# pythoncrazy/jimm

Hardware: AMD Instinct MI355X
Metric: images/sec (whole node) ViT-B/16@224 train (higher is better)
Workload: dtype bf16; 1 GPU; model=ViT-B/16@224, global_batch=1024, img_size=224, parallelism=dp1

## Files before the change

jimm_amd/csrc/attention.hip:

```cpp

#include <torch/extension.h>
#include <ATen/hip/HIPContext.h>

#include "mfma.h"

namespace {

constexpr int QBLK = 64;
constexpr int NSTRIP = 2;
constexpr int KVBLK = 64;


template <bool CAUSAL, int DP>
__global__ __launch_bounds__(256) void attn_fwd_kernel(
    const bf16* __restrict__ q, const bf16* __restrict__ k, const bf16* __restrict__ v,
    bf16* __restrict__ o, float* __restrict__ lse, int Lq, int Lk, float scale, int H, int Dr,
    hstride q_s, hstride k_s, hstride v_s, hstride o_s) {
  constexpr int LDS_PITCH = DP + 8;
  constexpr int NS = DP / 32;
  constexpr int NT = DP / 16;
  constexpr int IMGSF = KVBLK * LDS_PITCH + KVBLK * DP;
  extern __shared__ __attribute__((aligned(16))) char smem[];
  short* k_lds = reinterpret_cast<short*>(smem);
  short* vt_lds = k_lds + KVBLK * LDS_PITCH;
// ... 179 lines not shown
    float invl_r[4];
#pragma unroll
    for (int r = 0; r < 4; ++r) invl_r[r] = __shfl(invl, hi * 4 + r, WAVE);
#pragma unroll
    for (int r = 0; r < 4; ++r) {
      const int qrow = q0 + hi * 4 + r;
      if (qrow >= Lq) continue;
#pragma unroll
      for (int dt = 0; dt < NT; ++dt)
        if (DP == 64 || 16 * dt + lo < Dr)
          op[(int64_t)qrow * o_s.l + 16 * dt + lo] = f2bf(acc_o[st][dt][r] * invl_r[r]);
    }
    if (hi == 0 && q0 + lo < Lq)
      lse[bh * Lq + q0 + lo] = m_run[st] + __logf(l_run[st]);
  }
}


template <bool CAUSAL>
__global__ __launch_bounds__(320) void attn_fwd_small_kernel(
    const bf16* __restrict__ q, const bf16* __restrict__ k, const bf16* __restrict__ v,
    bf16* __restrict__ o, float* __restrict__ lse, int Lq, int Lk, float scale, int H,
    hstride q_s, hstride k_s, hstride v_s, hstride o_s) {
  constexpr int D = 64;
  constexpr int LP = 96;
  constexpr int PPITCH = 88;
  constexpr int PSTRIDE = 16 * PPITCH + 8;
  extern __shared__ __attribute__((aligned(16))) char smem[];
  const int wave = threadIdx.x / WAVE;
  const int lane = threadIdx.x % WAVE;
  const int lo = lane & 15, hi = lane >> 4;
  short* vb = reinterpret_cast<short*>(smem);
  short* pt = vb + LP * D + wave * PSTRIDE;

  const int64_t bh = blockIdx.x;
#pragma unroll
  for (int i = 0; i < (PSTRIDE / 8 + WAVE - 1) / WAVE; ++i) {
    const int idx = i * WAVE + lane;
    if (idx < PSTRIDE / 8) *reinterpret_cast<bf16x8*>(pt + idx * 8) = bf16x8{};
  }
  const bf16* qp = head_ptr(q, q_s, bh, H);
  const bf16* kp = head_ptr(k, k_s, bh, H);
  const bf16* vp = head_ptr(v, v_s, bh, H);
  bf16* op = head_ptr(o, o_s, bh, H);

  {
    const int t = (int)threadIdx.x;
    for (int idx = t; idx < LP * D / 8; idx += 320) {
      const int key = idx >> 3;
      const int d8 = (idx & 7) * 8;
      bf16x8 vv_{};
      if (key < Lk) vv_ = *reinterpret_cast<const bf16x8*>(vp + (int64_t)key * v_s.l + d8);
      *reinterpret_cast<bf16x8*>(vb + boff<D>(key, d8)) = vv_;
    }
  }
  const int nq = (Lq + 15) / 16;
  const int nkt = (Lk + 15) / 16;
  const int qs = wave;
  __syncthreads();
  if (qs < nq) {
    const int q0 = qs * 16;
    const int ktmax0 = CAUSAL ? min(nkt, qs + 1) : nkt;
    bf16x8 kfr[5][2];
#pragma unroll
    for (int kt = 0; kt < 5; ++kt) {
      const int key = 16 * kt + lo;
#pragma unroll
      for (int s = 0; s < 2; ++s)
        kfr[kt][s] = (kt < ktmax0 && key < Lk)
                         ? *reinterpret_cast<const bf16x8*>(kp + (int64_t)key * k_s.l + 32 * s + hi * 8)
                         : bf16x8{};
    }
    const int qrow = min(q0 + lo, Lq - 1);
    const bf16x8 qb0 = *reinterpret_cast<const bf16x8*>(qp + (int64_t)qrow * q_s.l + hi * 8);
    const bf16x8 qb1 = *reinterpret_cast<const bf16x8*>(qp + (int64_t)qrow * q_s.l + 32 + hi * 8);

    const int ktmax = ktmax0;
    f32x4 sc[5] = {};
    __builtin_amdgcn_s_setprio(1);
#pragma unroll
    for (int kt = 0; kt < 5; ++kt) {
      if (kt >= ktmax) continue;
      sc[kt] = MFMA16(kfr[kt][0], qb0, sc[kt]);
      sc[kt] = MFMA16(kfr[kt][1], qb1, sc[kt]);
    }
    __builtin_amdgcn_s_setprio(0);

    const int q_idx = q0 + lo;
    float sv[20];
#pragma unroll
    for (int kt = 0; kt < 5; ++kt) {
#pragma unroll
      for (int r = 0; r < 4; ++r) {
        const int key = 16 * kt + hi * 4 + r;
        float x = sc[kt][r] * scale;
        if (kt >= ktmax || key >= Lk || (CAUSAL && key > q_idx)) x = -INFINITY;
        sv[4 * kt + r] = x;
      }
    }
    float mt = sv[0];
#pragma unroll
    for (int i = 1; i < 20; ++i) mt = fmaxf(mt, sv[i]);
    mt = fmaxf(mt, __shfl_xor(mt, 16, WAVE));
    mt = fmaxf(mt, __shfl_xor(mt, 32, WAVE));
    float psum = 0.f;
#pragma unroll
    for (int i = 0; i < 20; ++i) {
      const float p = (sv[i] == -INFINITY) ? 0.f : __expf(sv[i] - mt);
      sv[i] = p;
      psum += p;
    }
    psum += __shfl_xor(psum, 16, WAVE);
    psum += __shfl_xor(psum, 32, WAVE);

#pragma unroll
    for (int kt = 0; kt < 5; ++kt) {
      bf16x4 pk;
#pragma unroll
      for (int r = 0; r < 4; ++r) pk[r] = f2bfs(sv[4 * kt + r]);
      *reinterpret_cast<bf16x4*>(pt + lo * PPITCH + 16 * kt + hi * 4) = pk;
    }

    f32x4 acc_o[4] = {};
    const int kv_hi = CAUSAL ? min(Lk, q0 + 16) : Lk;
#pragma unroll
    for (int s = 0; s < 3; ++s) {
      if (32 * s >= kv_hi) continue;
      bf16x8 vbf[4];
      const lds_cp bbase = (lds_cp)(const void*)(vb + s * 32 * D) + lane * 8;
      tr_frag_x4(bbase, vbf);
      const bf16x8 pa = row_frag(pt, lo, PPITCH, s, hi);
      __builtin_amdgcn_s_setprio(1);
#pragma unroll
      for (int dt = 0; dt < 4; ++dt) acc_o[dt] = MFMA16(pa, vbf[dt], acc_o[dt]);
      __builtin_amdgcn_s_setprio(0);
    }

    const float invl = psum > 0.f ? 1.f / psum : 0.f;
    float invl_r[4];
#pragma unroll
    for (int r = 0; r < 4; ++r) invl_r[r] = __shfl(invl, hi * 4 + r, WAVE);
#pragma unroll
    for (int r = 0; r < 4; ++r) {
      const int qr = q0 + hi * 4 + r;
      if (qr >= Lq) continue;
#pragma unroll
      for (int dt = 0; dt < 4; ++dt)
        op[(int64_t)qr * o_s.l + 16 * dt + lo] = f2bf(acc_o[dt][r] * invl_r[r]);
    }
    if (hi == 0 && q0 + lo < Lq) lse[bh * Lq + q0 + lo] = mt + __logf(psum);
  }
}

}

std::vector<torch::Tensor> attn_fwd(torch::Tensor q, torch::Tensor k, torch::Tensor v,
                                    bool causal, double scale) {
  check_attn_args("attn_fwd", {{"q", q}}, {{"k", k}, {"v", v}});
  const int Dr = q.size(3);
  const int DP = Dr <= 64 ? 64 : (Dr <= 96 ? 96 : 128);
  const int B = q.size(0), H = q.size(1), Lq = q.size(2), Lk = k.size(2);
  auto o = torch::empty({B, Lq, H, Dr}, q.options()).permute({0, 2, 1, 3});
  auto lse = torch::empty({B, H, Lq}, q.options().dtype(torch::kFloat32));
  const unsigned BH = (unsigned)((int64_t)B * H);
  auto stream = at::hip::getCurrentHIPStream();
  with_flags(
      [&](auto c) {
        constexpr bool C = decltype(c)::value;
        if (Dr == 64 && Lq == Lk && Lk <= 80) {
          const size_t shmem = (96 * 64 + 5 * (16 * 88 + 8)) * sizeof(short);
          launch_lds<attn_fwd_small_kernel<C>>(
              dim3(BH), dim3(320), shmem, shmem, stream, bf16_ptr(q), bf16_ptr(k), bf16_ptr(v),
              bf16_ptr(o), lse.data_ptr<float>(), Lq, Lk, (float)scale, H, hstrides(q),
              hstrides(k), hstrides(v), hstrides(o));
          return;
        }
        const int ntq = (Lq + QBLK - 1) / QBLK;
        const size_t shmem =
            (2 * (KVBLK * DP + KVBLK * (DP + 8)) + 4 * 16 * (DP + 8)) * sizeof(short);
        with_int<64, 96, 128>(DP, "padded head dim", [&](auto dp) {
          launch_lds<attn_fwd_kernel<C, decltype(dp)::value>>(
              dim3((ntq + NSTRIP - 1) / NSTRIP, BH), dim3(256), shmem, shmem, stream,
              bf16_ptr(q), bf16_ptr(k), bf16_ptr(v), bf16_ptr(o), lse.data_ptr<float>(), Lq, Lk,
              (float)scale, H, Dr, hstrides(q), hstrides(k), hstrides(v), hstrides(o));
        });
      },
      causal);
  return {o, lse};
}
```

jimm_amd/csrc/attention_bwd_fused.hip:

```cpp

#include <torch/extension.h>
#include <ATen/hip/HIPContext.h>

#include "mfma.h"

namespace {

constexpr int BLK = 64;

constexpr int tiles_per_wg(int DP) { return DP == 64 ? 2 : 1; }



__global__ void attn_d2_kernel(const bf16* __restrict__ dO, const bf16* __restrict__ O,
                               float* __restrict__ Dv, int H, int L, int Dr, int64_t nrows,
                               hstride do_s, hstride o_s) {
  const int wave = threadIdx.x / WAVE;
  const int lane = threadIdx.x % WAVE;
  const int wpb = blockDim.x / WAVE;
  const int sub = lane >> 3;
  const int c0 = (lane & 7) * 8;
  for (int64_t base = ((int64_t)blockIdx.x * wpb + wave) * 8; base < nrows;
       base += (int64_t)gridDim.x * wpb * 8) {
    const int64_t row = base + sub;
// ... 470 lines not shown
  const int64_t bh = blockIdx.x;
  const bf16* qp = head_ptr(q, q_s, bh, H);
  const bf16* kp = head_ptr(k, k_s, bh, H);
  const bf16* vp = head_ptr(v, v_s, bh, H);
  const bf16* dop = head_ptr(dO, do_s, bh, H);
  bf16* dqp = head_ptr(dq, dq_s, bh, H);
  bf16* dkp = head_ptr(dk, dk_s, bh, H);
  bf16* dvp = head_ptr(dv, dv_s, bh, H);

  for (int i = threadIdx.x; i < (3 * TILE + 8) / 8; i += 320)
    *reinterpret_cast<bf16x8*>(PT + i * 8) = bf16x8{};
  auto stage = [&](short* img, const bf16* src, int64_t sl, int rows) {
    for (int idx = (int)threadIdx.x; idx < IMG / 8; idx += 320) {
      const int row = idx >> 3, d8 = (idx & 7) * 8;
      bf16x8 vv{};
      if (row < rows) vv = *reinterpret_cast<const bf16x8*>(src + (int64_t)row * sl + d8);
      *reinterpret_cast<bf16x8*>(img + boff<D>(row, d8)) = vv;
    }
  };
  stage(imgA, kp, k_s.l, Lk);
  stage(imgQ, qp, q_s.l, Lq);
  stage(imgD, dop, do_s.l, Lq);
  const int nq = (Lq + 15) / 16;
  const int nkt = (Lk + 15) / 16;
  __syncthreads();

  if (wave < nq) {
    const int qs = wave;
    const int q0 = 16 * qs;
    const int ktmax = CAUSAL ? min(nkt, qs + 1) : nkt;
    bf16x8 kfr[5][2], vfr[5][2];
#pragma unroll
    for (int kt = 0; kt < 5; ++kt) {
      const int key = 16 * kt + lo;
      const bool ok = kt < ktmax && key < Lk;
#pragma unroll
      for (int sj = 0; sj < 2; ++sj) {
        kfr[kt][sj] = ok ? *reinterpret_cast<const bf16x8*>(
                               kp + (int64_t)key * k_s.l + 32 * sj + hi * 8)
                         : bf16x8{};
        vfr[kt][sj] = ok ? *reinterpret_cast<const bf16x8*>(
                               vp + (int64_t)key * v_s.l + 32 * sj + hi * 8)
                         : bf16x8{};
      }
    }
    const int qrow = min(q0 + lo, Lq - 1);
    const bf16x8 qb0 = *reinterpret_cast<const bf16x8*>(qp + (int64_t)qrow * q_s.l + hi * 8);
    const bf16x8 qb1 =
        *reinterpret_cast<const bf16x8*>(qp + (int64_t)qrow * q_s.l + 32 + hi * 8);
    const bf16x8 db0 =
        *reinterpret_cast<const bf16x8*>(dop + (int64_t)qrow * do_s.l + hi * 8);
    const bf16x8 db1 =
        *reinterpret_cast<const bf16x8*>(dop + (int64_t)qrow * do_s.l + 32 + hi * 8);
    f32x4 sc[5] = {}, dpc[5] = {};
    __builtin_amdgcn_s_setprio(1);
#pragma unroll
    for (int kt = 0; kt < 5; ++kt) {
      if (kt >= ktmax) continue;
      sc[kt] = MFMA16(kfr[kt][0], qb0, sc[kt]);
      sc[kt] = MFMA16(kfr[kt][1], qb1, sc[kt]);
      dpc[kt] = MFMA16(vfr[kt][0], db0, dpc[kt]);
      dpc[kt] = MFMA16(vfr[kt][1], db1, dpc[kt]);
    }
    __builtin_amdgcn_s_setprio(0);
    const int q_idx = q0 + lo;
    const float lse_q = lse[bh * Lq + qrow];
    float pv[20];
    float dsum = 0.f;
#pragma unroll
    for (int kt = 0; kt < 5; ++kt) {
#pragma unroll
      for (int r = 0; r < 4; ++r) {
        const int key = 16 * kt + 4 * hi + r;
        const bool ok =
            kt < ktmax && key < Lk && q_idx < Lq && (!CAUSAL || key <= q_idx);
        const float p = ok ? __expf(sc[kt][r] * scale - lse_q) : 0.f;
        pv[4 * kt + r] = p;
        dsum += p * dpc[kt][r];
      }
    }
    dsum += __shfl_xor(dsum, 16, WAVE);
    dsum += __shfl_xor(dsum, 32, WAVE);
#pragma unroll
    for (int kt = 0; kt < 5; ++kt) {
      bf16x4 ds4;
#pragma unroll
      for (int r = 0; r < 4; ++r) {
        const int key = 16 * kt + 4 * hi + r;
        const float p = pv[4 * kt + r];
        const float ds = p * (dpc[kt][r] - dsum) * scale;
        PT[key * TP + q_idx] = f2bfs(p);
        DST[key * TP + q_idx] = f2bfs(ds);
        ds4[r] = f2bfs(ds);
      }
      *reinterpret_cast<bf16x4*>(DSQ + q_idx * TP + 16 * kt + 4 * hi) = ds4;
    }
    f32x4 adq[4] = {};
    const int smax = (16 * ktmax + 31) / 32;
#pragma unroll
    for (int sb = 0; sb < 3; ++sb) {
      if (sb >= smax) continue;
      bf16x8 bfr[4];
      tr_frag_x4((lds_cp)(const void*)(imgA + sb * 32 * D) + lane * 8, bfr);
      const bf16x8 pa = row_frag(DSQ, q0 + lo, TP, sb, hi);
      __builtin_amdgcn_s_setprio(1);
#pragma unroll
      for (int dt = 0; dt < 4; ++dt) adq[dt] = MFMA16(pa, bfr[dt], adq[dt]);
      __builtin_amdgcn_s_setprio(0);
    }
#pragma unroll
    for (int r = 0; r < 4; ++r) {
      const int qr = q0 + 4 * hi + r;
      if (qr >= Lq) continue;
#pragma unroll
      for (int dt = 0; dt < 4; ++dt)
        dqp[(int64_t)qr * dq_s.l + 16 * dt + lo] = f2bf(adq[dt][r]);
    }
  }
  __syncthreads();

  if (wave < nkt) {
    const int k0 = 16 * wave;
    const int smin = CAUSAL ? k0 / 32 : 0;
    const int nsq = (Lq + 31) / 32;
    f32x4 adk[4] = {}, adv[4] = {};
    for (int sb = smin; sb < nsq; ++sb) {
      bf16x8 bq[4], bd[4];
      tr_frag_x4((lds_cp)(const void*)(imgQ + sb * 32 * D) + lane * 8, bq);
      tr_frag_x4((lds_cp)(const void*)(imgD + sb * 32 * D) + lane * 8, bd);
      const bf16x8 ak = row_frag(DST, k0 + lo, TP, sb, hi);
      const bf16x8 av = row_frag(PT, k0 + lo, TP, sb, hi);
      __builtin_amdgcn_s_setprio(1);
#pragma unroll
      for (int dt = 0; dt < 4; ++dt) {
        adk[dt] = MFMA16(ak, bq[dt], adk[dt]);
        adv[dt] = MFMA16(av, bd[dt], adv[dt]);
      }
      __builtin_amdgcn_s_setprio(0);
    }
#pragma unroll
    for (int r = 0; r < 4; ++r) {
      const int kr = k0 + 4 * hi + r;
      if (kr >= Lk) continue;
#pragma unroll
      for (int dt = 0; dt < 4; ++dt) {
        dkp[(int64_t)kr * dk_s.l + 16 * dt + lo] = f2bf(adk[dt][r]);
        dvp[(int64_t)kr * dv_s.l + 16 * dt + lo] = f2bf(adv[dt][r]);
      }
    }
  }
}


constexpr int RES_LMIN = 81;
constexpr int RES_LMAX = 256;

__device__ __forceinline__ int noff(int row, int d) {
  return (row >> 5) * 2048 + (d >> 4) * 512 + (row & 31) * 16 + (d & 15);
}

__global__ __launch_bounds__(512, 4) void attn_bwd_resident_kernel(
    const bf16* __restrict__ q, const bf16* __restrict__ k, const bf16* __restrict__ v,
    const bf16* __restrict__ o, const bf16* __restrict__ dO, const float* __restrict__ lse,
    bf16* __restrict__ dq, bf16* __restrict__ dk, bf16* __restrict__ dv, int L, float scale,
    int H, hstride q_s, hstride k_s, hstride v_s, hstride o_s, hstride do_s, hstride dq_s,
    hstride dk_s, hstride dv_s) {
  constexpr int D = 64;
  extern __shared__ __attribute__((aligned(16))) char smem[];
  const int LP = (L + 31) & ~31;
  const int IMG = LP * D;
  short* imgA = reinterpret_cast<short*>(smem);
  short* imgB = imgA + IMG;
  float* lse_s = reinterpret_cast<float*>(imgB + IMG);
  float* dl_s = lse_s + LP;

  const int tid = threadIdx.x;
  const int nthr = blockDim.x;
  const int nw = nthr / WAVE;
  const int wave = tid / WAVE;
  const int lane = tid % WAVE;
  const int lo = lane & 15, hi = lane >> 4;
  const int64_t bh = blockIdx.x;
  const bf16* qp = head_ptr(q, q_s, bh, H);
  const bf16* kp = head_ptr(k, k_s, bh, H);
  const bf16* vp = head_ptr(v, v_s, bh, H);
  const bf16* op = head_ptr(o, o_s, bh, H);
  const bf16* dop = head_ptr(dO, do_s, bh, H);
  const int nblk = LP / 32;

  bf16x8 qb[2], dob[2];
  float dl;
  auto load_rows = [&](int s0) {
    const int srow = min(s0 + lo, L - 1);
    dl = 0.f;
#pragma unroll
    for (int s = 0; s < 2; ++s) {
      qb[s] = *reinterpret_cast<const bf16x8*>(qp + (int64_t)srow * q_s.l + 32 * s + hi * 8);
      dob[s] = *reinterpret_cast<const bf16x8*>(dop + (int64_t)srow * do_s.l + 32 * s + hi * 8);
      const bf16x8 ov =
          *reinterpret_cast<const bf16x8*>(op + (int64_t)srow * o_s.l + 32 * s + hi * 8);
#pragma unroll
      for (int j = 0; j < 8; ++j) dl += bfs2f(dob[s][j]) * bfs2f(ov[j]);
    }
    dl += __shfl_xor(dl, 16, WAVE);
    dl += __shfl_xor(dl, 32, WAVE);
  };
  load_rows(16 * wave);

#pragma unroll
  for (int it = 0; it < 4; ++it) {
    const int idx = tid + it * nthr;
    const int row = idx >> 3, d8 = (idx & 7) * 8;
    const int rc = min(row, L - 1);
    bf16x8 kk = *reinterpret_cast<const bf16x8*>(kp + (int64_t)rc * k_s.l + d8);
    bf16x8 vv = *reinterpret_cast<const bf16x8*>(vp + (int64_t)rc * v_s.l + d8);
    if (row >= L) kk = vv = bf16x8{};
    const int off = noff(row, d8);
    *reinterpret_cast<bf16x8*>(imgA + off) = kk;
    *reinterpret_cast<bf16x8*>(imgB + off) = vv;
  }
  for (int i = tid; i < LP; i += nthr) {
    lse_s[i] = i < L ? lse[bh * L + i] : 0.f;
    dl_s[i] = 0.f;
  }
  __syncthreads();

#pragma unroll
  for (int i = 0; i < 2; ++i) {
    const int s0 = 16 * (wave + i * nw);
    if (s0 >= L) continue;
    if (i == 1) load_rows(s0);
    const bool sok = s0 + lo < L;
    const float lse_q = lse_s[min(s0 + lo, L - 1)];
    const float dli = dl;
    if (hi == 0) dl_s[s0 + lo] = dli;
    f32x4 adq[4] = {};
    for (int kb = 0; kb < nblk; ++kb) {
      f32x4 sc[2] = {}, dpc[2] = {};
#pragma unroll
      for (int t = 0; t < 2; ++t) {
        if (32 * kb + 16 * t >= L) continue;
        bf16x8 ka[2], va[2];
#pragma unroll
        for (int s = 0; s < 2; ++s) {
          const int off = noff(32 * kb + 16 * t + lo, 32 * s + hi * 8);
          ka[s] = *reinterpret_cast<const bf16x8*>(imgA + off);
          va[s] = *reinterpret_cast<const bf16x8*>(imgB + off);
        }
        __builtin_amdgcn_s_setprio(1);
#pragma unroll
        for (int s = 0; s < 2; ++s) {
          sc[t] = MFMA16(ka[s], qb[s], sc[t]);
          dpc[t] = MFMA16(va[s], dob[s], dpc[t]);
        }
        __builtin_amdgcn_s_setprio(0);
      }
      bf16x8 dsa;
#pragma unroll
      for (int t = 0; t < 2; ++t) {
#pragma unroll
        for (int r = 0; r < 4; ++r) {
          const int key = 32 * kb + 16 * t + 4 * hi + r;
          const bool ok = sok && key < L;
          const float p = ok ? __expf(sc[t][r] * scale - lse_q) : 0.f;
          const float ds = ok ? p * (dpc[t][r] - dli) * scale : 0.f;
          dsa[4 * t + r] = f2bfs(ds);
        }
      }
      bf16x8 bfr[4];
      tr_frag_x4((lds_cp)(const void*)(imgA + kb * 32 * D) + lane * 8, bfr);
      __builtin_amdgcn_s_setprio(1);
#pragma unroll
      for (int dt = 0; dt < 4; ++dt) adq[dt] = MFMA16(bfr[dt], dsa, adq[dt]);
      __builtin_amdgcn_s_setprio(0);
    }
    if (sok) {
      bf16* dqp = head_ptr(dq, dq_s, bh, H) + (int64_t)(s0 + lo) * dq_s.l + 4 * hi;
#pragma unroll
      for (int dt = 0; dt < 4; ++dt) {
        bf16x4 pk;
#pragma unroll
        for (int r = 0; r < 4; ++r) pk[r] = f2bfs(adq[dt][r]);
        *reinterpret_cast<bf16x4*>(dqp + 16 * dt) = pk;
      }
    }
  }

  bf16x8 qst[4], dst[4];
#pragma unroll
  for (int it = 0; it < 4; ++it) {
    const int idx = tid + it * nthr;
    const int row = idx >> 3, d8 = (idx & 7) * 8;
    const int rc = min(row, L - 1);
    qst[it] = *reinterpret_cast<const bf16x8*>(qp + (int64_t)rc * q_s.l + d8);
    dst[it] = *reinterpret_cast<const bf16x8*>(dop + (int64_t)rc * do_s.l + d8);
    if (row >= L) qst[it] = dst[it] = bf16x8{};
  }
  bf16x8 kbf[2][2], vbf[2][2];
#pragma unroll
  for (int i = 0; i < 2; ++i) {
    const int srow = min(16 * (wave + i * nw) + lo, LP - 1);
#pragma unroll
    for (int s = 0; s < 2; ++s) {
      const int off = noff(srow, 32 * s + hi * 8);
      kbf[i][s] = *reinterpret_cast<const bf16x8*>(imgA + off);
      vbf[i][s] = *reinterpret_cast<const bf16x8*>(imgB + off);
    }
  }
  __syncthreads();
#pragma unroll
  for (int it = 0; it < 4; ++it) {
    const int idx = tid + it * nthr;
    const int off = noff(idx >> 3, (idx & 7) * 8);
    *reinterpret_cast<bf16x8*>(imgA + off) = qst[it];
    *reinterpret_cast<bf16x8*>(imgB + off) = dst[it];
  }
  __syncthreads();

#pragma unroll
  for (int i = 0; i < 2; ++i) {
    const int s0 = 16 * (wave + i * nw);
    if (s0 >= L) continue;
    const bool sok = s0 + lo < L;
    f32x4 adk[4] = {}, adv[4] = {};
    for (int qblk = 0; qblk < nblk; ++qblk) {
      f32x4 sc[2] = {}, dpc[2] = {};
#pragma unroll
      for (int t = 0; t < 2; ++t) {
        if (32 * qblk + 16 * t >= L) continue;
        bf16x8 qa[2], da[2];
#pragma unroll
        for (int s = 0; s < 2; ++s) {
          const int off = noff(32 * qblk + 16 * t + lo, 32 * s + hi * 8);
          qa[s] = *reinterpret_cast<const bf16x8*>(imgA + off);
          da[s] = *reinterpret_cast<const bf16x8*>(imgB + off);
        }
        __builtin_amdgcn_s_setprio(1);
#pragma unroll
        for (int s = 0; s < 2; ++s) {
          sc[t] = MFMA16(qa[s], kbf[i][s], sc[t]);
          dpc[t] = MFMA16(da[s], vbf[i][s], dpc[t]);
        }
        __builtin_amdgcn_s_setprio(0);
      }
      bf16x8 pa, dsa;
#pragma unroll
      for (int t = 0; t < 2; ++t) {
        const int qi0 = 32 * qblk + 16 * t + 4 * hi;
        const f32x4 ls4 = *reinterpret_cast<const f32x4*>(lse_s + qi0);
        const f32x4 dl4 = *reinterpret_cast<const f32x4*>(dl_s + qi0);
#pragma unroll
        for (int r = 0; r < 4; ++r) {
          const bool ok = sok && qi0 + r < L;
          const float p = ok ? __expf(sc[t][r] * scale - ls4[r]) : 0.f;
          const float ds = ok ? p * (dpc[t][r] - dl4[r]) * scale : 0.f;
          pa[4 * t + r] = f2bfs(p);
          dsa[4 * t + r] = f2bfs(ds);
        }
      }
      bf16x8 bfr[4];
      tr_frag_x4((lds_cp)(const void*)(imgB + qblk * 32 * D) + lane * 8, bfr);
      __builtin_amdgcn_s_setprio(1);
#pragma unroll
      for (int dt = 0; dt < 4; ++dt) adv[dt] = MFMA16(bfr[dt], pa, adv[dt]);
      __builtin_amdgcn_s_setprio(0);
      tr_frag_x4((lds_cp)(const void*)(imgA + qblk * 32 * D) + lane * 8, bfr);
      __builtin_amdgcn_s_setprio(1);
#pragma unroll
      for (int dt = 0; dt < 4; ++dt) adk[dt] = MFMA16(bfr[dt], dsa, adk[dt]);
      __builtin_amdgcn_s_setprio(0);
    }
    if (sok) {
      bf16* dkp = head_ptr(dk, dk_s, bh, H) + (int64_t)(s0 + lo) * dk_s.l + 4 * hi;
      bf16* dvp = head_ptr(dv, dv_s, bh, H) + (int64_t)(s0 + lo) * dv_s.l + 4 * hi;
#pragma unroll
      for (int dt = 0; dt < 4; ++dt) {
        bf16x4 pk, pv;
#pragma unroll
        for (int r = 0; r < 4; ++r) {
          pk[r] = f2bfs(adk[dt][r]);
          pv[r] = f2bfs(adv[dt][r]);
        }
        *reinterpret_cast<bf16x4*>(dkp + 16 * dt) = pk;
        *reinterpret_cast<bf16x4*>(dvp + 16 * dt) = pv;
      }
    }
  }
}

}

void attn_bwd_fused(torch::Tensor q, torch::Tensor k, torch::Tensor v, torch::Tensor o,
                    torch::Tensor dO, torch::Tensor lse, torch::Tensor dq, torch::Tensor dk,
                    torch::Tensor dv, bool causal, double scale, std::string path) {
  check_attn_args("attn_bwd_fused", {{"q", q}, {"o", o}, {"dO", dO}, {"dq", dq}},
                  {{"k", k}, {"v", v}, {"dk", dk}, {"dv", dv}}, &lse);
  const int Dr = q.size(3);
  const int DP = Dr <= 64 ? 64 : (Dr <= 96 ? 96 : 128);
  const int B = q.size(0), H = q.size(1), Lq = q.size(2), Lk = k.size(2);
  const unsigned BH = (unsigned)((int64_t)B * H);
  auto stream = at::hip::getCurrentHIPStream();

  TORCH_CHECK(path == "auto" || path == "tiled" || path == "resident",
              "attn_bwd_fused: path must be auto, tiled or resident, got ", path);
  bool res_aligned = true;
  for (auto* t : {&q, &k, &v, &o, &dO, &dq, &dk, &dv})
    res_aligned = res_aligned && reinterpret_cast<uintptr_t>(t->data_ptr()) % 16 == 0 &&
                  t->stride(0) % 8 == 0 && t->stride(1) % 8 == 0 && t->stride(2) % 8 == 0;
  const bool resident_ok = Dr == 64 && Lq == Lk && !causal && Lk >= RES_LMIN &&
                           Lk <= RES_LMAX && res_aligned;
  TORCH_CHECK(path != "resident" || resident_ok,
              "attn_bwd_fused: path=resident needs D == 64, Lq == Lk, non-causal, ",
              RES_LMIN, " <= L <= ", RES_LMAX, " and 16-byte aligned rows; got D=", Dr,
              " Lq=", Lq, " Lk=", Lk, " causal=", causal, " aligned=", res_aligned);
  if (path != "tiled" && resident_ok) {
    const int LP = (Lk + 31) & ~31;
    const size_t rshmem = (size_t)2 * LP * 64 * sizeof(short) + (size_t)2 * LP * sizeof(float);
    constexpr size_t rshmem_max =
        (size_t)2 * RES_LMAX * 64 * sizeof(short) + (size_t)2 * RES_LMAX * sizeof(float);
    launch_lds<attn_bwd_resident_kernel>(
        dim3(BH), dim3(LP / 32 * WAVE), rshmem, rshmem_max, stream, bf16_ptr(q), bf16_ptr(k),
        bf16_ptr(v), bf16_ptr(o), bf16_ptr(dO), lse.data_ptr<float>(), bf16_ptr(dq),
        bf16_ptr(dk), bf16_ptr(dv), Lk, (float)scale, H, hstrides(q), hstrides(k), hstrides(v),
        hstrides(o), hstrides(dO), hstrides(dq), hstrides(dk), hstrides(dv));
    return;
  }

  if (path != "tiled" && Dr == 64 && Lq == Lk && Lk <= 80) {
    const size_t shmem = (3 * 96 * 64 + 3 * 80 * 88 + 8) * sizeof(short);
    with_flags(
        [&](auto c) {
          launch_lds<attn_bwd_small_kernel<decltype(c)::value>>(
              dim3(BH), dim3(320), shmem, shmem, stream, bf16_ptr(q), bf16_ptr(k), bf16_ptr(v),
              bf16_ptr(dO), lse.data_ptr<float>(), bf16_ptr(dq), bf16_ptr(dk), bf16_ptr(dv), Lq,
              Lk, (float)scale, H, hstrides(q), hstrides(k), hstrides(v), hstrides(dO),
              hstrides(dq), hstrides(dk), hstrides(dv));
        },
        causal);
    return;
  }

  auto Dv = torch::empty({(int64_t)B * H * Lq}, q.options().dtype(torch::kFloat32));
  {
    const int64_t nrows = (int64_t)B * H * Lq;
    const dim3 grid((unsigned)std::min<int64_t>((nrows + 3) / 4, 4096));
    hipLaunchKernelGGL(attn_d2_kernel, grid, dim3(256), 0, stream, bf16_ptr(dO), bf16_ptr(o),
                       Dv.data_ptr<float>(), H, Lq, Dr, nrows, hstrides(dO), hstrides(o));
  }

  const int pitch = DP + 8;
  const size_t shmem_dkv =
      (2 * (2 * BLK * DP + 2 * BLK * pitch) + 4 * 16 * pitch) * sizeof(short);
  const size_t shmem_dq = (2 * (BLK * DP + 2 * BLK * pitch) + 4 * 16 * pitch) * sizeof(short);
  const int ntk = (Lk + BLK - 1) / BLK;
  const int ntq = (Lq + BLK - 1) / BLK;
  const int tpw = tiles_per_wg(DP);
  with_flags(
      [&](auto c) {
        with_int<64, 96, 128>(DP, "padded head dim", [&](auto dp) {
          constexpr bool C = decltype(c)::value;
          constexpr int P = decltype(dp)::value;
          launch_lds<attn_bwd_dkv_kernel<C, P>>(
              dim3((ntk + tpw - 1) / tpw, BH), dim3(256), shmem_dkv, shmem_dkv, stream,
              bf16_ptr(q), bf16_ptr(k), bf16_ptr(v), bf16_ptr(dO), lse.data_ptr<float>(),
              Dv.data_ptr<float>(), bf16_ptr(dk), bf16_ptr(dv), Lq, Lk, (float)scale, H, Dr,
              hstrides(q), hstrides(k), hstrides(v), hstrides(dO), hstrides(dk), hstrides(dv));
          launch_lds<attn_bwd_dq_kernel<C, P>>(
              dim3((ntq + tpw - 1) / tpw, BH), dim3(256), shmem_dq, shmem_dq, stream,
              bf16_ptr(q), bf16_ptr(k), bf16_ptr(v), bf16_ptr(dO), lse.data_ptr<float>(),
              Dv.data_ptr<float>(), bf16_ptr(dq), Lq, Lk, (float)scale, H, Dr, hstrides(q),
              hstrides(k), hstrides(v), hstrides(dO), hstrides(dq));
        });
      },
      causal);
}
```

jimm_amd/csrc/bindings.cpp:

```cpp

#include <torch/extension.h>

std::vector<torch::Tensor> layernorm_fwd(torch::Tensor x, torch::Tensor w, torch::Tensor b, double eps);
std::vector<torch::Tensor> layernorm_bwd(torch::Tensor dy, torch::Tensor x, torch::Tensor w,
                                         torch::Tensor mean, torch::Tensor rstd,
                                         c10::optional<torch::Tensor> addend);
torch::Tensor bias_act_fwd(torch::Tensor z, c10::optional<torch::Tensor> bias, std::string act,
                           c10::optional<torch::Tensor> residual);
std::vector<torch::Tensor> bias_act_fwd_fp8(torch::Tensor z, c10::optional<torch::Tensor> bias,
                                            std::string act, torch::Tensor scale8,
                                            torch::Tensor amax);
std::vector<torch::Tensor> gemm_nt_8p_gradact_fp8(torch::Tensor dy, torch::Tensor wt,
                                                  torch::Tensor z, std::string act,
                                                  torch::Tensor scale8, torch::Tensor amax);
std::vector<torch::Tensor> layernorm_fwd_fp8(torch::Tensor x, torch::Tensor w, torch::Tensor b,
                                             double eps, torch::Tensor scale8,
                                             torch::Tensor amax);
torch::Tensor act_bwd(torch::Tensor dy, torch::Tensor z, std::string act);
torch::Tensor colsum(torch::Tensor dz);
torch::Tensor im2col_patch(torch::Tensor img, int64_t patch);
torch::Tensor cls_pos_fwd(torch::Tensor x, c10::optional<torch::Tensor> cls, torch::Tensor pos);
torch::Tensor embed_pos_fwd(torch::Tensor ids, torch::Tensor emb, torch::Tensor pos);
torch::Tensor col2im_patch(torch::Tensor cols, std::vector<int64_t> img_shape, int64_t patch);
void adam_step(std::vector<torch::Tensor> ps, std::vector<torch::Tensor> gs,
               std::vector<torch::Tensor> ms, std::vector<torch::Tensor> vs,
               std::vector<c10::optional<torch::Tensor>> masters, double lr, double b1,
               double b2, double eps, double wd, int64_t step);
std::vector<torch::Tensor> adam_prepare(std::vector<torch::Tensor> ps,
                                        std::vector<torch::Tensor> gs,
                                        std::vector<torch::Tensor> ms,
                                        std::vector<torch::Tensor> vs,
                                        std::vector<c10::optional<torch::Tensor>> masters);
void adam_apply(torch::Tensor desc, int64_t nchunks, torch::Tensor lr_dev,
                torch::Tensor step_dev, double b1, double b2, double eps, double wd);
std::vector<torch::Tensor> attn_fwd(torch::Tensor q, torch::Tensor k, torch::Tensor v,
                                    bool causal, double scale);
void attn_bwd_p(torch::Tensor s, torch::Tensor lse, bool causal, double scale);
torch::Tensor attn_d(torch::Tensor dO, torch::Tensor O);
void attn_ds(torch::Tensor dp, torch::Tensor p, torch::Tensor D, double scale);
void attn_bwd_fused(torch::Tensor q, torch::Tensor k, torch::Tensor v, torch::Tensor o,
                    torch::Tensor dO, torch::Tensor lse, torch::Tensor dq, torch::Tensor dk,
                    torch::Tensor dv, bool causal, double scale, std::string path);
torch::Tensor mfma_probe(torch::Tensor A, torch::Tensor B);
torch::Tensor mfma_probe32(torch::Tensor A, torch::Tensor B);
bool gemm_supported(int64_t M, int64_t N, int64_t K, std::string dtype);
std::vector<torch::Tensor> l2norm_fwd(torch::Tensor x);
torch::Tensor l2norm_bwd(torch::Tensor dy, torch::Tensor x, torch::Tensor rinv);
std::vector<torch::Tensor> xent_rows_fwd(torch::Tensor logits, torch::Tensor labels);
torch::Tensor xent_rows_bwd(torch::Tensor logits, torch::Tensor labels, torch::Tensor lse,
                            double gscale);
std::vector<torch::Tensor> sigmoid_loss_ew(torch::Tensor logits, int64_t diag0);
bool gemm8p_supported(int64_t M, int64_t N, int64_t K);
bool gemm_tn8p_supported(int64_t M, int64_t N, int64_t K);
int64_t gemm_tn8p_choose_splitm(int64_t M, int64_t tiles, int64_t cus);
torch::Tensor gemm_tn_8p(torch::Tensor dz, torch::Tensor x, int64_t splitm, bool out_bf16);
std::vector<torch::Tensor> gemm_tn_8p_db(torch::Tensor dz, torch::Tensor x, int64_t splitm,
                                         bool out_bf16);
torch::Tensor gemm_nt_8p_gradact(torch::Tensor dy, torch::Tensor wt, torch::Tensor z, std::string act);
torch::Tensor tr16_probe(torch::Tensor src, int64_t mode);
std::vector<torch::Tensor> linear_fwd(torch::Tensor x, torch::Tensor w,
                                      c10::optional<torch::Tensor> bias, std::string act,
                                      c10::optional<torch::Tensor> residual, bool save_z);
std::vector<torch::Tensor> linear_fwd_actgrad(torch::Tensor x, torch::Tensor w,
                                              c10::optional<torch::Tensor> bias,
                                              std::string act,
                                              c10::optional<torch::Tensor> residual);
torch::Tensor gemm_nt_8p_gradmul(torch::Tensor dy, torch::Tensor wt, torch::Tensor g);

PYBIND11_MODULE(TORCH_EXTENSION_NAME, m) {
  m.def("layernorm_fwd", &layernorm_fwd, "LayerNorm forward (K3)");
  m.def("layernorm_bwd", &layernorm_bwd, "LayerNorm backward (K3/K15), optional fused addend",
        py::arg("dy"), py::arg("x"), py::arg("w"), py::arg("mean"), py::arg("rstd"),
        py::arg("addend") = py::none());
  m.def("bias_act_fwd", &bias_act_fwd, "fused bias+activation(+residual) forward");
  m.def("bias_act_fwd_fp8", &bias_act_fwd_fp8, "bias+act forward with fused e4m3 emit");
  m.def("gemm_nt_8p_gradact_fp8", &gemm_nt_8p_gradact_fp8,
        "gradact dX GEMM with fused e4m3 emit of dz");
  m.def("layernorm_fwd_fp8", &layernorm_fwd_fp8, "LayerNorm forward with fused e4m3 emit");
  m.def("act_bwd", &act_bwd, "activation backward: dy * act'(z)");
  m.def("colsum", &colsum, "column sum -> fp32 (bias gradient, K15)");
  m.def("im2col_patch", &im2col_patch, "patch-embed unfold (K1)");
  m.def("cls_pos_fwd", &cls_pos_fwd, "fused CLS concat + pos-emb add (K2)");
  m.def("embed_pos_fwd", &embed_pos_fwd, "fused token-embed gather + pos-emb add (K10)");
  m.def("col2im_patch", &col2im_patch, "patch-embed fold backward (K1/K15)");
  m.def("adam_step", &adam_step, "fused multi-tensor Adam (K14)");
  m.def("adam_prepare", &adam_prepare, "build device chunk descriptors once (K14)");
  m.def("adam_apply", &adam_apply, "graph-capturable fused Adam update (K14)");
  m.def("attn_fwd", &attn_fwd, "flash attention forward, head_dim 64 (K5)");
  m.def("attn_bwd_p", &attn_bwd_p, "attention bwd: S -> P in place (K15)");
  m.def("attn_d", &attn_d, "attention bwd: rowsum(dO*O) (K15)");
  m.def("attn_ds", &attn_ds, "attention bwd: dP -> dS in place (K15)");
  m.def("attn_bwd_fused", &attn_bwd_fused,
        "fused flash attention backward (K15); path: auto | tiled | resident",
        py::arg("q"), py::arg("k"), py::arg("v"), py::arg("o"), py::arg("dO"), py::arg("lse"),
        py::arg("dq"), py::arg("dk"), py::arg("dv"), py::arg("causal"), py::arg("scale"),
        py::arg("path") = "auto");
  m.def("mfma_probe", &mfma_probe, "MFMA 16x16x32 layout probe");
  m.def("mfma_probe32", &mfma_probe32, "MFMA 32x32x16 layout probe");
  m.def("gemm_supported", &gemm_supported, "MFMA GEMM shape support check");
  m.def("gemm8p_supported", &gemm8p_supported, "8-phase 256-tile GEMM shape check");
  m.def("gemm_tn8p_supported", &gemm_tn8p_supported, "TN dW GEMM shape check");
  m.def("gemm_tn8p_choose_splitm", &gemm_tn8p_choose_splitm,
        "TN dW split-M heuristic (host only)", py::arg("M"), py::arg("tiles"), py::arg("cus"));
  m.def("gemm_tn_8p", &gemm_tn_8p, "TN weight-grad GEMM, split-M, tr_b16 (K15)",
        py::arg("dz"), py::arg("x"), py::arg("splitm") = 0, py::arg("out_bf16") = false);
  m.def("gemm_tn_8p_db", &gemm_tn_8p_db, "split-M TN dW with fused bias-grad colsum",
        py::arg("dz"), py::arg("x"), py::arg("splitm") = 0, py::arg("out_bf16") = false);
  m.def("gemm_nt_8p_gradact", &gemm_nt_8p_gradact, "dX GEMM with fused act-backward epilogue");
  m.def("tr16_probe", &tr16_probe, "ds_read_b64_tr_b16 lane-mapping probe");
  m.def("l2norm_fwd", &l2norm_fwd, "row L2-normalize forward (K12)");
  m.def("l2norm_bwd", &l2norm_bwd, "row L2-normalize backward (K12)");
  m.def("xent_rows_fwd", &xent_rows_fwd, "fused softmax-CE forward (K13)");
  m.def("xent_rows_bwd", &xent_rows_bwd, "fused softmax-CE backward (K13)");
  m.def("sigmoid_loss_ew", &sigmoid_loss_ew, "SigLIP sigmoid loss + dLogits (K13)");
  m.def("linear_fwd", &linear_fwd, "MFMA GEMM + fused epilogue (K4/K6/K7/K8)");
  m.def("linear_fwd_actgrad", &linear_fwd_actgrad,
        "linear_fwd that returns (y, fp16 act'(pre)) instead of the pre-activation",
        py::arg("x"), py::arg("w"), py::arg("bias"), py::arg("act"),
        py::arg("residual") = py::none());
  m.def("gemm_nt_8p_gradmul", &gemm_nt_8p_gradmul,
        "dX GEMM times a saved fp16 activation derivative");
}
```

jimm_amd/csrc/mfma.h:

```cpp
#pragma once

#include <string>
#include <type_traits>

#include "common.h"

#define MFMA16(A, B, C) __builtin_amdgcn_mfma_f32_16x16x32_bf16(A, B, C, 0, 0, 0)


__device__ __forceinline__ void raw_barrier() {
  asm volatile("s_barrier" ::: "memory");
}

__device__ __forceinline__ void glds16(const bf16* g, char* lds_dst) {
  typedef const __attribute__((address_space(1))) unsigned int* gp_t;
  typedef __attribute__((address_space(3))) unsigned int* lp_t;
  __builtin_amdgcn_global_load_lds((gp_t)(const void*)g, (lp_t)(void*)lds_dst, 16, 0, 0);
}

__device__ __forceinline__ int xcd_remap(int wg, int nwg) {
  const int q = nwg / 8, r = nwg % 8;
  const int xcd = wg % 8, idx = wg / 8;
  return (xcd < r ? xcd * (q + 1) : r * (q + 1) + (xcd - r) * q) + idx;
}

template <int DP>
__device__ __forceinline__ bf16x8 ld8g(const bf16* p, int off, int Dr) {
  if (DP == 64 || off + 8 <= Dr) return *reinterpret_cast<const bf16x8*>(p + off);
  return bf16x8{};
}

template <int ND>
__device__ __forceinline__ int boff(int q, int d) {
  const int qp = (q >> 2) & 7;
  const int qpos = (qp & 1) * 4 + (qp >> 1);
  return (q >> 5) * (32 * ND) + (d >> 4) * 512 + qpos * 64 + (q & 3) * 16 + (d & 15);
}

typedef const __attribute__((address_space(3))) char* lds_cp;

__device__ __forceinline__ void tr_frag_x4(lds_cp base, bf16x8 (&out)[4]) {
  bf16x4 a0l, a0h, a1l, a1h, a2l, a2h, a3l, a3h;
  asm volatile(
      "ds_read_b64_tr_b16 %0, %8 offset:0\n\t"
      "ds_read_b64_tr_b16 %1, %8 offset:512\n\t"
      "ds_read_b64_tr_b16 %2, %8 offset:1024\n\t"
      "ds_read_b64_tr_b16 %3, %8 offset:1536\n\t"
      "ds_read_b64_tr_b16 %4, %8 offset:2048\n\t"
      "ds_read_b64_tr_b16 %5, %8 offset:2560\n\t"
      "ds_read_b64_tr_b16 %6, %8 offset:3072\n\t"
      "ds_read_b64_tr_b16 %7, %8 offset:3584\n\t"
      "s_waitcnt lgkmcnt(0)"
      : "=&v"(a0l), "=&v"(a0h), "=&v"(a1l), "=&v"(a1h), "=&v"(a2l), "=&v"(a2h),
        "=&v"(a3l), "=&v"(a3h)
      : "v"(base)
      : "memory");
  __builtin_amdgcn_sched_barrier(0);
  out[0] = __builtin_shufflevector(a0l, a0h, 0, 1, 2, 3, 4, 5, 6, 7);
  out[1] = __builtin_shufflevector(a1l, a1h, 0, 1, 2, 3, 4, 5, 6, 7);
  out[2] = __builtin_shufflevector(a2l, a2h, 0, 1, 2, 3, 4, 5, 6, 7);
  out[3] = __builtin_shufflevector(a3l, a3h, 0, 1, 2, 3, 4, 5, 6, 7);
}

__device__ __forceinline__ void tr_frag_x2(lds_cp base, bf16x8 (&out)[2]) {
  bf16x4 a0l, a0h, a1l, a1h;
  asm volatile(
      "ds_read_b64_tr_b16 %0, %4 offset:0\n\t"
      "ds_read_b64_tr_b16 %1, %4 offset:512\n\t"
      "ds_read_b64_tr_b16 %2, %4 offset:1024\n\t"
      "ds_read_b64_tr_b16 %3, %4 offset:1536\n\t"
      "s_waitcnt lgkmcnt(0)"
      : "=&v"(a0l), "=&v"(a0h), "=&v"(a1l), "=&v"(a1h)
      : "v"(base)
      : "memory");
  __builtin_amdgcn_sched_barrier(0);
  out[0] = __builtin_shufflevector(a0l, a0h, 0, 1, 2, 3, 4, 5, 6, 7);
  out[1] = __builtin_shufflevector(a1l, a1h, 0, 1, 2, 3, 4, 5, 6, 7);
}

template <int NT>
__device__ __forceinline__ void tr_frags(lds_cp base, bf16x8 (&out)[NT]) {
  static_assert(NT == 4 || NT == 6 || NT == 8, "head dims 64, 96, 128");
  tr_frag_x4(base, *reinterpret_cast<bf16x8(*)[4]>(&out[0]));
  if constexpr (NT == 6) tr_frag_x2(base + 4096, *reinterpret_cast<bf16x8(*)[2]>(&out[4]));
  if constexpr (NT == 8) tr_frag_x4(base + 4096, *reinterpret_cast<bf16x8(*)[4]>(&out[4]));
}

__device__ __forceinline__ bf16x8 row_frag(const short* img, int row, int pitch, int step,
                                           int hi) {
  return *reinterpret_cast<const bf16x8*>(img + row * pitch + 32 * step + hi * 8);
}


struct hstride {
  int64_t b, h, l;
};

template <typename T>
__device__ __forceinline__ T* head_ptr(T* base, const hstride& s, int64_t bh, int H) {
  return base + (bh / H) * s.b + (bh % H) * s.h;
}


#define SAVE_NONE 0
#define SAVE_PRE 1
#define SAVE_GRAD 2

#define GRADM_NONE 0
#define GRADM_ACT 1
#define GRADM_MUL 2

__device__ __forceinline__ float load_bias(const void* bias, int n, int bias_bf16) {
  return bias_bf16 ? bf2f(static_cast<const bf16*>(bias)[n])
                   : static_cast<const float*>(bias)[n];
}

template <int ACT, bool HAS_BIAS, bool HAS_RES, int SAVE, int GRADM = GRADM_NONE,
          bool FP8O = false>
__device__ __forceinline__ void gemm_epilogue(float vpre, int m, int n, int N, float bias_n,
                                              const bf16* res, bf16* Y, bf16* Z,
                                              unsigned char* Y8 = nullptr, float rs8 = 1.f,
                                              float* tmax = nullptr) {
  static_assert(SAVE != SAVE_GRAD || ACT != ACT_NONE, "SAVE_GRAD needs an activation");
  if (HAS_BIAS) vpre += bias_n;
  if (SAVE == SAVE_PRE) Z[(int64_t)m * N + n] = f2bf(vpre);
  float vy;
  if (GRADM == GRADM_ACT) {
    vy = vpre * act_grad(bf2f(res[(int64_t)m * N + n]), ACT);
  } else if (GRADM == GRADM_MUL) {
    vy = vpre * __half2float(reinterpret_cast<const __half*>(res)[(int64_t)m * N + n]);
  } else {
    if (SAVE == SAVE_GRAD) {
      float g;
      vy = act_fwd_grad(vpre, ACT, &g);
      reinterpret_cast<__half*>(Z)[(int64_t)m * N + n] = __float2half(g);
    } else {
      vy = act_fwd(vpre, ACT);
    }
    if (HAS_RES) vy += bf2f(res[(int64_t)m * N + n]);
  }
  Y[(int64_t)m * N + n] = f2bf(vy);
  if (FP8O) {
    *tmax = fmaxf(*tmax, fabsf(vy));
    Y8[(int64_t)m * N + n] = cvt_e4m3(vy * rs8);
  }
}


int act_code(const std::string& act);

template <int... Vs, typename F>
void with_int(int v, const char* what, F&& f) {
  const bool found = ((v == Vs ? (f(std::integral_constant<int, Vs>{}), true) : false) || ...);
  TORCH_CHECK(found, "bad ", what, " ", v);
}

template <typename F>
void with_act(int act, F&& f) {
  with_int<ACT_NONE, ACT_GELU, ACT_GELU_TANH, ACT_QUICKGELU>(act, "activation code", f);
}

template <typename F>
void with_save(int save, F&& f) {
  with_int<SAVE_NONE, SAVE_PRE, SAVE_GRAD>(save, "save mode", f);
}

template <typename F>
void with_flags(F&& f) {
  f();
}
template <typename F, typename... Rest>
void with_flags(F&& f, bool b, Rest... rest) {
  if (b) with_flags([&](auto... cs) { f(std::true_type{}, cs...); }, rest...);
  else with_flags([&](auto... cs) { f(std::false_type{}, cs...); }, rest...);
}

template <auto Kernel, typename... Args>
void launch_lds(dim3 grid, dim3 block, size_t shmem, size_t shmem_limit, hipStream_t stream,
                Args... args) {
  static const bool raised = [&] {
    HIP_CHECK(hipFuncSetAttribute(reinterpret_cast<const void*>(Kernel),
                                  hipFuncAttributeMaxDynamicSharedMemorySize,
                                  (int)shmem_limit));
    return true;
  }();
  (void)raised;
  hipLaunchKernelGGL(Kernel, grid, block, shmem, stream, args...);
}


inline hstride hstrides(const torch::Tensor& t) {
  return {t.stride(0), t.stride(1), t.stride(2)};
}

inline bf16* bf16_ptr(const torch::Tensor& t) {
  return reinterpret_cast<bf16*>(t.data_ptr());
}

struct named_tensor {
  const char* name;
  const torch::Tensor& t;
};

inline void check_attn_args(const char* op, std::initializer_list<named_tensor> q_like,
                            std::initializer_list<named_tensor> k_like,
                            const torch::Tensor* lse = nullptr) {
  const torch::Tensor& q = q_like.begin()->t;
  const torch::Tensor& k = k_like.begin()->t;
  for (const auto* list : {&q_like, &k_like}) {
    const torch::Tensor& first = list->begin()->t;
    for (const named_tensor& n : *list) {
      TORCH_CHECK(n.t.is_cuda(), op, ": ", n.name, " must be a CUDA tensor");
      TORCH_CHECK(n.t.scalar_type() == torch::kBFloat16, op, ": ", n.name,
                  " must be bf16, got ", n.t.scalar_type());
      TORCH_CHECK(n.t.dim() == 4, op, ": ", n.name, " must be (B,H,L,D), got ", n.t.dim(),
                  " dims");
      TORCH_CHECK(n.t.stride(3) == 1, op, ": innermost dim of ", n.name,
                  " must be contiguous");
      TORCH_CHECK(n.t.sizes() == first.sizes(), op, ": ", n.name, " has shape ", n.t.sizes(),
                  ", expected ", list->begin()->name, "'s ", first.sizes());
    }
  }
  const int64_t D = q.size(3);
  TORCH_CHECK(D == 64 || D == 72 || D == 80 || D == 96 || D == 128, op,
              ": head_dim must be one of {64,72,80,96,128}, got ", D);
  TORCH_CHECK(k.size(0) == q.size(0) && k.size(1) == q.size(1) && k.size(3) == D, op,
              ": k has shape ", k.sizes(), ", expected q's B, H and D ", q.sizes());
  if (lse) {
    TORCH_CHECK(lse->is_cuda() && lse->is_contiguous() &&
                    lse->scalar_type() == torch::kFloat32 &&
                    lse->numel() == q.size(0) * q.size(1) * q.size(2),
                op, ": lse must be contiguous fp32 (B,H,Lq)");
  }
}
```

Measured before the change: 6610 images/sec.

## Add LDS-resident single-pass attention forward kernel for short sequences

Adds a forward attention kernel that loads a head's full K and V into LDS once and computes exact softmax in a single pass per 16-row query strip, with no online rescaling. It is used by default when head dim is 64, the sequence is non-causal and 81 to 256 long (ViT-B/16 has 197 tokens). The aim is to drop the tiled flash loop's repeated KV loads, running-max rescaling and multi-block bookkeeping. In exchange it keeps more score registers live, and occupancy is bounded by the LDS used for whole-head K and V. Shared helpers move into the common header.

Result: faster. 6757 images/sec, median of 6 (+2.2%).

```diff
diff --git a/jimm_amd/csrc/attention.hip b/jimm_amd/csrc/attention.hip
--- a/jimm_amd/csrc/attention.hip
+++ b/jimm_amd/csrc/attention.hip
@@ -355,18 +355,168 @@
   }
 }
 
+
+template <int NBLK>
+__global__ __launch_bounds__(512, 4) void attn_fwd_resident_kernel(
+    const bf16* __restrict__ q, const bf16* __restrict__ k, const bf16* __restrict__ v,
+    bf16* __restrict__ o, float* __restrict__ lse, int L, float scale, int H, hstride q_s,
+    hstride k_s, hstride v_s, hstride o_s) {
+  constexpr int D = 64;
+  constexpr int LP = 32 * NBLK;
+  constexpr int IMG = LP * D;
+  constexpr int NTHR = 64 * NBLK;
+  extern __shared__ __attribute__((aligned(16))) char smem[];
+  short* imgK = reinterpret_cast<short*>(smem);
+  short* imgV = imgK + IMG;
+
+  const int tid = threadIdx.x;
+  const int wave = tid / WAVE;
+  const int lane = tid % WAVE;
+  const int lo = lane & 15, hi = lane >> 4;
+  const int64_t bh = blockIdx.x;
+  const bf16* qp = head_ptr(q, q_s, bh, H);
+  const bf16* kp = head_ptr(k, k_s, bh, H);
+  const bf16* vp = head_ptr(v, v_s, bh, H);
+
+  bf16x8 qb[2][2];
+#pragma unroll
+  for (int i = 0; i < 2; ++i) {
+    const int srow = min(16 * (wave + i * NBLK) + lo, L - 1);
+#pragma unroll
+    for (int s = 0; s < 2; ++s)
+      qb[i][s] = *reinterpret_cast<const bf16x8*>(qp + (int64_t)srow * q_s.l + 32 * s + hi * 8);
+  }
+
+#pragma unroll
+  for (int it = 0; it < 4; ++it) {
+    const int idx = tid + it * NTHR;
+    const int row = idx >> 3, d8 = (idx & 7) * 8;
+    const int rc = min(row, L - 1);
+    bf16x8 kk = *reinterpret_cast<const bf16x8*>(kp + (int64_t)rc * k_s.l + d8);
+    bf16x8 vv = *reinterpret_cast<const bf16x8*>(vp + (int64_t)rc * v_s.l + d8);
+    if (row >= L) kk = vv = bf16x8{};
+    const int off = noff(row, d8);
+    *reinterpret_cast<bf16x8*>(imgK + off) = kk;
+    *reinterpret_cast<bf16x8*>(imgV + off) = vv;
+  }
+  __syncthreads();
+
+  const float c = scale * 1.44269504088896340736f;
+#pragma unroll
+  for (int i = 0; i < 2; ++i) {
+    const int s0 = 16 * (wave + i * NBLK);
+    if (s0 >= L) continue;
+    const bool sok = s0 + lo < L;
+
+    f32x4 sc[NBLK][2];
+#pragma unroll
+    for (int kb = 0; kb < NBLK; ++kb) {
+#pragma unroll
+      for (int t = 0; t < 2; ++t) {
+        sc[kb][t] = f32x4{};
+        if (kb == NBLK - 1 && 32 * kb + 16 * t >= L) continue;
+        bf16x8 ka[2];
+#pragma unroll
+        for (int s = 0; s < 2; ++s)
+          ka[s] = *reinterpret_cast<const bf16x8*>(
+              imgK + noff(32 * kb + 16 * t + lo, 32 * s + hi * 8));
+        __builtin_amdgcn_s_setprio(1);
+#pragma unroll
+        for (int s = 0; s < 2; ++s) sc[kb][t] = MFMA16(ka[s], qb[i][s], sc[kb][t]);
+        __builtin_amdgcn_s_setprio(0);
+      }
+    }
+
+    float m = -INFINITY;
+#pragma unroll
+    for (int kb = 0; kb < NBLK; ++kb) {
+#pragma unroll
+      for (int t = 0; t < 2; ++t) {
+#pragma unroll
+        for (int r = 0; r < 4; ++r) {
+          float x = sc[kb][t][r] * c;
+          if (kb == NBLK - 1 && 32 * kb + 16 * t + 4 * hi + r >= L) x = -INFINITY;
+          sc[kb][t][r] = x;
+          m = fmaxf(m, x);
+        }
+      }
+    }
+    m = fmaxf(m, __shfl_xor(m, 16, WAVE));
+    m = fmaxf(m, __shfl_xor(m, 32, WAVE));
+    const float msub = sok ? m : INFINITY;
+
+    float lsum = 0.f;
+    f32x4 acc[4] = {};
+#pragma unroll
+    for (int kb = 0; kb < NBLK; ++kb) {
+      bf16x8 pf;
+#pragma unroll
+      for (int t = 0; t < 2; ++t) {
+#pragma unroll
+        for (int r = 0; r < 4; ++r) {
+          const float p = __builtin_amdgcn_exp2f(sc[kb][t][r] - msub);
+          lsum += p;
+          pf[4 * t + r] = f2bfs(p);
+        }
+      }
+      bf16x8 vfr[4];
+      tr_frag_x4((lds_cp)(const void*)(imgV + kb * 32 * D) + lane * 8, vfr);
+      __builtin_amdgcn_s_setprio(1);
+#pragma unroll
+      for (int dt = 0; dt < 4; ++dt) acc[dt] = MFMA16(vfr[dt], pf, acc[dt]);
+      __builtin_amdgcn_s_setprio(0);
+    }
+    lsum += __shfl_xor(lsum, 16, WAVE);
+    lsum += __shfl_xor(lsum, 32, WAVE);
+
+    if (sok) {
+      const float invl = 1.f / lsum;
+      bf16* op = head_ptr(o, o_s, bh, H) + (int64_t)(s0 + lo) * o_s.l + 4 * hi;
+#pragma unroll
+      for (int dt = 0; dt < 4; ++dt) {
+        bf16x4 pk;
+#pragma unroll
+        for (int r = 0; r < 4; ++r) pk[r] = f2bfs(acc[dt][r] * invl);
+        *reinterpret_cast<bf16x4*>(op + 16 * dt) = pk;
+      }
+      if (hi == 0) lse[bh * L + s0 + lo] = m * 0.69314718055994530942f + __logf(lsum);
+    }
+  }
 }
 
+}
+
 std::vector<torch::Tensor> attn_fwd(torch::Tensor q, torch::Tensor k, torch::Tensor v,
-                                    bool causal, double scale) {
+                                    bool causal, double scale, std::string path) {
   check_attn_args("attn_fwd", {{"q", q}}, {{"k", k}, {"v", v}});
   const int Dr = q.size(3);
   const int DP = Dr <= 64 ? 64 : (Dr <= 96 ? 96 : 128);
   const int B = q.size(0), H = q.size(1), Lq = q.size(2), Lk = k.size(2);
+  TORCH_CHECK(path == "auto" || path == "tiled" || path == "resident",
+              "attn_fwd: path must be auto, tiled or resident, got ", path);
+  const bool aligned = res_aligned({&q, &k, &v});
+  const bool resident_ok = Dr == 64 && Lq == Lk && !causal && Lk >= RES_LMIN &&
+                           Lk <= RES_LMAX && aligned;
+  TORCH_CHECK(path != "resident" || resident_ok,
+              "attn_fwd: path=resident needs D == 64, Lq == Lk, non-causal, ", RES_LMIN,
+              " <= L <= ", RES_LMAX, " and 16-byte aligned rows; got D=", Dr, " Lq=", Lq,
+              " Lk=", Lk, " causal=", causal, " aligned=", aligned);
   auto o = torch::empty({B, Lq, H, Dr}, q.options()).permute({0, 2, 1, 3});
   auto lse = torch::empty({B, H, Lq}, q.options().dtype(torch::kFloat32));
   const unsigned BH = (unsigned)((int64_t)B * H);
   auto stream = at::hip::getCurrentHIPStream();
+  if (path != "tiled" && resident_ok) {
+    const int nblk = (Lk + 31) / 32;
+    const size_t rshmem = (size_t)2 * nblk * 32 * 64 * sizeof(short);
+    constexpr size_t rshmem_max = (size_t)2 * RES_LMAX * 64 * sizeof(short);
+    with_int<3, 4, 5, 6, 7, 8>(nblk, "resident block count", [&](auto nb) {
+      launch_lds<attn_fwd_resident_kernel<decltype(nb)::value>>(
+          dim3(BH), dim3(nblk * WAVE), rshmem, rshmem_max, stream, bf16_ptr(q), bf16_ptr(k),
+          bf16_ptr(v), bf16_ptr(o), lse.data_ptr<float>(), Lk, (float)scale, H, hstrides(q),
+          hstrides(k), hstrides(v), hstrides(o));
+    });
+    return {o, lse};
+  }
   with_flags(
       [&](auto c) {
         constexpr bool C = decltype(c)::value;
diff --git a/jimm_amd/csrc/attention_bwd_fused.hip b/jimm_amd/csrc/attention_bwd_fused.hip
--- a/jimm_amd/csrc/attention_bwd_fused.hip
+++ b/jimm_amd/csrc/attention_bwd_fused.hip
@@ -646,13 +646,6 @@
 }
 
 
-constexpr int RES_LMIN = 81;
-constexpr int RES_LMAX = 256;
-
-__device__ __forceinline__ int noff(int row, int d) {
-  return (row >> 5) * 2048 + (d >> 4) * 512 + (row & 31) * 16 + (d & 15);
-}
-
 __global__ __launch_bounds__(512, 4) void attn_bwd_resident_kernel(
     const bf16* __restrict__ q, const bf16* __restrict__ k, const bf16* __restrict__ v,
     const bf16* __restrict__ o, const bf16* __restrict__ dO, const float* __restrict__ lse,
@@ -897,16 +890,13 @@
 
   TORCH_CHECK(path == "auto" || path == "tiled" || path == "resident",
               "attn_bwd_fused: path must be auto, tiled or resident, got ", path);
-  bool res_aligned = true;
-  for (auto* t : {&q, &k, &v, &o, &dO, &dq, &dk, &dv})
-    res_aligned = res_aligned && reinterpret_cast<uintptr_t>(t->data_ptr()) % 16 == 0 &&
-                  t->stride(0) % 8 == 0 && t->stride(1) % 8 == 0 && t->stride(2) % 8 == 0;
+  const bool aligned = res_aligned({&q, &k, &v, &o, &dO, &dq, &dk, &dv});
   const bool resident_ok = Dr == 64 && Lq == Lk && !causal && Lk >= RES_LMIN &&
-                           Lk <= RES_LMAX && res_aligned;
+                           Lk <= RES_LMAX && aligned;
   TORCH_CHECK(path != "resident" || resident_ok,
               "attn_bwd_fused: path=resident needs D == 64, Lq == Lk, non-causal, ",
               RES_LMIN, " <= L <= ", RES_LMAX, " and 16-byte aligned rows; got D=", Dr,
-              " Lq=", Lq, " Lk=", Lk, " causal=", causal, " aligned=", res_aligned);
+              " Lq=", Lq, " Lk=", Lk, " causal=", causal, " aligned=", aligned);
   if (path != "tiled" && resident_ok) {
     const int LP = (Lk + 31) & ~31;
     const size_t rshmem = (size_t)2 * LP * 64 * sizeof(short) + (size_t)2 * LP * sizeof(float);
diff --git a/jimm_amd/csrc/bindings.cpp b/jimm_amd/csrc/bindings.cpp
--- a/jimm_amd/csrc/bindings.cpp
+++ b/jimm_amd/csrc/bindings.cpp
@@ -34,7 +34,7 @@
 void adam_apply(torch::Tensor desc, int64_t nchunks, torch::Tensor lr_dev,
                 torch::Tensor step_dev, double b1, double b2, double eps, double wd);
 std::vector<torch::Tensor> attn_fwd(torch::Tensor q, torch::Tensor k, torch::Tensor v,
-                                    bool causal, double scale);
+                                    bool causal, double scale, std::string path);
 void attn_bwd_p(torch::Tensor s, torch::Tensor lse, bool causal, double scale);
 torch::Tensor attn_d(torch::Tensor dO, torch::Tensor O);
 void attn_ds(torch::Tensor dp, torch::Tensor p, torch::Tensor D, double scale);
@@ -86,7 +86,10 @@
   m.def("adam_step", &adam_step, "fused multi-tensor Adam (K14)");
   m.def("adam_prepare", &adam_prepare, "build device chunk descriptors once (K14)");
   m.def("adam_apply", &adam_apply, "graph-capturable fused Adam update (K14)");
-  m.def("attn_fwd", &attn_fwd, "flash attention forward, head_dim 64 (K5)");
+  m.def("attn_fwd", &attn_fwd,
+        "flash attention forward (K5); path: auto | tiled | resident",
+        py::arg("q"), py::arg("k"), py::arg("v"), py::arg("causal"), py::arg("scale"),
+        py::arg("path") = "auto");
   m.def("attn_bwd_p", &attn_bwd_p, "attention bwd: S -> P in place (K15)");
   m.def("attn_d", &attn_d, "attention bwd: rowsum(dO*O) (K15)");
   m.def("attn_ds", &attn_ds, "attention bwd: dP -> dS in place (K15)");
diff --git a/jimm_amd/csrc/mfma.h b/jimm_amd/csrc/mfma.h
--- a/jimm_amd/csrc/mfma.h
+++ b/jimm_amd/csrc/mfma.h
@@ -99,6 +99,14 @@
 template <typename T>
 __device__ __forceinline__ T* head_ptr(T* base, const hstride& s, int64_t bh, int H) {
   return base + (bh / H) * s.b + (bh % H) * s.h;
+}
+
+
+constexpr int RES_LMIN = 81;
+constexpr int RES_LMAX = 256;
+
+__device__ __forceinline__ int noff(int row, int d) {
+  return (row >> 5) * 2048 + (d >> 4) * 512 + (row & 31) * 16 + (d & 15);
 }
 
 
@@ -197,6 +205,14 @@
   return reinterpret_cast<bf16*>(t.data_ptr());
 }
 
+inline bool res_aligned(std::initializer_list<const torch::Tensor*> ts) {
+  bool ok = true;
+  for (const torch::Tensor* t : ts)
+    ok = ok && reinterpret_cast<uintptr_t>(t->data_ptr()) % 16 == 0 && t->stride(0) % 8 == 0 &&
+         t->stride(1) % 8 == 0 && t->stride(2) % 8 == 0;
+  return ok;
+}
+
 struct named_tensor {
   const char* name;
   const torch::Tensor& t;
```
